# igashov/DiffLinker

Measured on NVIDIA H100. Metric: molecules/sec (T=500 denoising), higher is better.
Workload: dtype f32

## Files before the change

difflinker_b200/csrc/kernels_node_tc.cuh:

```cuda
#pragma once
#include "kernels_tc.cuh"

namespace dl {
namespace tcn {

using namespace dl::tc;

constexpr int TM = 128;
constexpr int X_LBO = TM * 16 + 16;
constexpr int X_BYTES = KC * X_LBO;
constexpr int HALF_BYTES = 8 * W_LBO;
constexpr int STAGE_BYTES = 2 * HALF_BYTES;
constexpr int BLOCK_BYTES = 2 * W_BYTES;
constexpr int N_RING = 2;
constexpr int N_OFF_WS = 4 * X_BYTES;
constexpr int N_OFF_MISC = N_OFF_WS + N_RING * STAGE_BYTES;
constexpr int N_OFF_BAR = N_OFF_MISC + 128 * 4 + 64;
constexpr int N_SMEM_BYTES = N_OFF_BAR + 64 + 1024;
static_assert(N_SMEM_BYTES <= 232448, "k_node_tc shared memory");
constexpr int NW = 8;
constexpr int W_NLOADER = NW;
constexpr int NODE_TC_THREADS = 32 * (NW + 1);

struct NodeTcArgs {
  float* h;
  const float* agg;
  const float* nm;
  const __half* w3;
  const __half* w4;
  const float *b3, *b4;
  float w3_descale, w4_descale;
  int tile_nodes;
  int proj_only;
  int n_proj;
  const __half* pw[2];
  const float* pb1[2];
  float p_descale[2];
  float* AB[2];
  float* ABmax[2];
};

__device__ __forceinline__ float pow2_scale_for(float bound) {
  float sc = 1.0f;
  if (!(bound <= F16_TARGET)) {
    const int ex = ((__float_as_int(bound) >> 23) & 0xff) - 127;
    sc = __int_as_float(max(127 + 13 - ex, 1) << 23);
  }
  return sc;
}

__device__ __forceinline__ void workers_sync() { asm volatile("bar.sync 1, %0;" ::"n"(32 * NW) : "memory"); }

__device__ __forceinline__ void store_elem(uint8_t* xhi, uint8_t* xlo, int c, int n, float v) {
  const __half hi = __float2half_rn(v);
  const __half lo = __float2half_rn(v - __half2float(hi));
  const int off = (c >> 3) * X_LBO + n * 16 + (c & 7) * 2;
  *reinterpret_cast<__half*>(xhi + off) = hi;
  *reinterpret_cast<__half*>(xlo + off) = lo;
}

__global__ void __launch_bounds__(NODE_TC_THREADS, 1) k_node_tc(int n_total, NodeTcArgs a) {
  extern __shared__ uint8_t smem_raw[];
  uint8_t* sm = smem_raw + ((1024u - (smem_u32(smem_raw) & 1023u)) & 1023u);
  const uint32_t sbase = smem_u32(sm);
  const int tid = threadIdx.x, warp = tid >> 5, lane = tid & 31;
  const int tile = a.tile_nodes > 0 ? a.tile_nodes : TM;
  const int g0 = blockIdx.x * tile;
  const int n_live = min(tile, n_total - g0);

  const uint32_t bar_full = sbase + N_OFF_BAR, bar_empty = bar_full + 8 * N_RING;
  uint8_t* xa_hi = sm; uint8_t* xa_lo = xa_hi + X_BYTES;
  uint8_t* xb_hi = sm + 2 * X_BYTES; uint8_t* xb_lo = xb_hi + X_BYTES;
  float* nms = reinterpret_cast<float*>(sm + N_OFF_MISC);
  int* tilemax = reinterpret_cast<int*>(sm + N_OFF_MISC + 512);

  if (tid == 0) {
    for (int i = 0; i < N_RING; ++i) { mbar_init(bar_full + 8 * i, 1); mbar_init(bar_empty + 8 * i, NW); }
    fence_barrier_init();
  }
  if (tid < 16) tilemax[tid] = 0;
  __syncthreads();

  const int blk0 = a.proj_only ? 3 : 0;
  const int n_blocks = 3 + 2 * a.n_proj - blk0;
  const int n_half = 2 * n_blocks;

  if (warp == W_NLOADER) {
    if (lane == 0) {
      for (int i = 0; i < n_half; ++i) {
        const int s = i % N_RING, blk = (i >> 1) + blk0, hf = i & 1;
        if (i >= N_RING) mbar_wait(bar_empty + 8 * s, ((i - N_RING) / N_RING) & 1);
        const __half* base = blk < 2 ? a.w3 + (size_t)blk * (BLOCK_BYTES / 2)
                             : blk == 2 ? a.w4
                                        : a.pw[(blk - 3) >> 1] + (size_t)((blk - 3) & 1) * (BLOCK_BYTES / 2);
        const uint8_t* src = reinterpret_cast<const uint8_t*>(base);
        const uint32_t dst = sbase + N_OFF_WS + s * STAGE_BYTES;
        mbar_expect_tx(bar_full + 8 * s, STAGE_BYTES);
        bulk_g2s(dst, src + hf * HALF_BYTES, HALF_BYTES, bar_full + 8 * s);
        bulk_g2s(dst + HALF_BYTES, src + W_BYTES + hf * HALF_BYTES, HALF_BYTES, bar_full + 8 * s);
      }
    }
    return;
  }

  chain_wait();
  if (tid == 0) chain_release();
  if (tid < TM) nms[tid] = tid < n_live ? a.nm[g0 + tid] : 0.f;

  const int g = warp >> 2, q = lane & 3;
  const int c0 = 64 * g + 16 * (warp & 3) + (lane >> 2);
  int tm_calls = 0;
  auto tile_max = [&](float mx) -> float {
#pragma unroll
    for (int o = 16; o > 0; o >>= 1) mx = fmaxf(mx, __shfl_xor_sync(0xffffffffu, mx, o));
    int* slot = tilemax + (tm_calls++ & 15);
    if (lane == 0) atomicMax(slot, __float_as_int(mx));
    workers_sync();
    return __int_as_float(*slot);
  };
  auto operand_ready = [&]() {
    fence_proxy_async();
    workers_sync();
  };
  int hb = 0;
  float d[64];
#pragma unroll
  for (int i = 0; i < 64; ++i) d[i] = 0.f;
  auto gemm = [&](const uint8_t* xop, int n_blk_half, bool accumulate) {
    for (int k = 0; k < n_blk_half; ++k, ++hb) {
      const int s = hb % N_RING, hf = hb & 1;
      mbar_wait(bar_full + 8 * s, (hb / N_RING) & 1);
      const uint32_t xh = smem_u32(xop) + (8 * hf) * X_LBO, xl = xh + X_BYTES;
      const uint32_t wh = sbase + N_OFF_WS + s * STAGE_BYTES + g * 1024, wl = wh + HALF_BYTES;
      gemm_3xf16(d, wh, wl, W_LBO, xh, xl, X_LBO, 2 * X_LBO, 4, accumulate || k > 0);
      __syncwarp();
      if (lane == 0) mbar_arrive(bar_empty + 8 * s);
    }
  };

  auto load_rows = [&](float scale) -> float {
    float mx = 0.f;
#pragma unroll 1
    for (int rb = warp; rb < TM; rb += 4 * NW) {
      float4 hv[4], av[4];
#pragma unroll
      for (int j = 0; j < 4; ++j) {
        const int r = rb + NW * j;
        hv[j] = make_float4(0, 0, 0, 0); av[j] = hv[j];
        if (r < n_live) {
          hv[j] = *reinterpret_cast<const float4*>(a.h + (size_t)(g0 + r) * H + lane * 4);
          if (!a.proj_only) av[j] = __ldg(reinterpret_cast<const float4*>(a.agg + (size_t)(g0 + r) * H + lane * 4));
        }
      }
#pragma unroll
      for (int j = 0; j < 4; ++j) {
        const int r = rb + NW * j;
        mx = fmaxf(mx, fmaxf(fmaxf(fabsf(hv[j].x), fabsf(hv[j].y)), fmaxf(fabsf(hv[j].z), fabsf(hv[j].w))));
        mx = fmaxf(mx, fmaxf(fmaxf(fabsf(av[j].x), fabsf(av[j].y)), fmaxf(fabsf(av[j].z), fabsf(av[j].w))));
        const int off = (lane >> 1) * X_LBO + r * 16 + (lane & 1) * 8;
        uint2 hi, lo;
        split2(hv[j].x * scale, hv[j].y * scale, hi.x, lo.x); split2(hv[j].z * scale, hv[j].w * scale, hi.y, lo.y);
        *reinterpret_cast<uint2*>(xa_hi + off) = hi; *reinterpret_cast<uint2*>(xa_lo + off) = lo;
        split2(av[j].x * scale, av[j].y * scale, hi.x, lo.x); split2(av[j].z * scale, av[j].w * scale, hi.y, lo.y);
        *reinterpret_cast<uint2*>(xb_hi + off) = hi; *reinterpret_cast<uint2*>(xb_lo + off) = lo;
      }
    }
    return mx;
  };

  float s1 = 1.f, s2 = 1.f, s3 = 1.f;
#pragma unroll 1
  for (int pass = 0; pass < 2; ++pass) {
    const float mx = load_rows(s1);
    if (pass == 1) break;
    s1 = pow2_scale_for(tile_max(mx));
    if (s1 == 1.0f) break;
  }
  operand_ready();

  if (a.proj_only) {
    s3 = s1;
  } else {
    gemm(xa_hi, 2, false);
    gemm(xb_hi, 2, true);
    workers_sync();
    const float2 bias3 = make_float2(__ldg(a.b3 + c0), __ldg(a.b3 + c0 + 8));
    const float ds1 = a.w3_descale / s1;
#pragma unroll 1
    for (int pass = 0; pass < 2; ++pass) {
      float mx = 0.f;
#pragma unroll
      for (int j = 0; j < 16; ++j)
#pragma unroll
        for (int u = 0; u < 4; ++u) {
          const float v = fmaf(d[4 * j + u], ds1, (u & 2) ? bias3.y : bias3.x);
          mx = fmaxf(mx, fabsf(v));
          store_elem(xb_hi, xb_lo, c0 + (u & 2) * 4, 8 * j + 2 * q + (u & 1), silu_f(v) * s2);
        }
      if (pass == 1) break;
      s2 = pow2_scale_for(tile_max(mx));
      if (s2 == 1.0f) break;
    }
    operand_ready();
    gemm(xb_hi, 2, false);
    const float2 bias4 = make_float2(__ldg(a.b4 + c0), __ldg(a.b4 + c0 + 8));
    const float ds2 = a.w4_descale / s2;
    float mx = 0.f;
#pragma unroll
    for (int j = 0; j < 16; ++j)
#pragma unroll
      for (int u = 0; u < 4; ++u) {
        const int n = 8 * j + 2 * q + (u & 1), c = c0 + (u & 2) * 4;
        float* hp = a.h + (size_t)(g0 + n) * H + c;
        const float hv = n < n_live ? *hp : 0.f;
        const float o = (hv + fmaf(d[4 * j + u], ds2, (u & 2) ? bias4.y : bias4.x)) * nms[n];
        if (n < n_live) *hp = o;
        mx = fmaxf(mx, fabsf(o));
        d[4 * j + u] = o;
        store_elem(xa_hi, xa_lo, c, n, o);
      }
    s3 = pow2_scale_for(tile_max(mx));
    if (s3 != 1.0f) {
#pragma unroll
      for (int j = 0; j < 16; ++j)
#pragma unroll
        for (int u = 0; u < 4; ++u) store_elem(xa_hi, xa_lo, c0 + (u & 2) * 4, 8 * j + 2 * q + (u & 1), d[4 * j + u] * s3);
    }
    operand_ready();
  }

  for (int p = 0; p < a.n_proj; ++p) {
#pragma unroll 1
    for (int pt = 0; pt < 2; ++pt) {
      gemm(xa_hi, 2, false);
      const float2 bias = pt == 0 ? make_float2(__ldg(a.pb1[p] + c0), __ldg(a.pb1[p] + c0 + 8)) : make_float2(0.f, 0.f);
      float* ab = a.AB[p] + (size_t)g0 * 2 * H + pt * H;
      const float ds = a.p_descale[p] / s3;
      float mx = 0.f;
#pragma unroll
      for (int j = 0; j < 16; ++j)
#pragma unroll
        for (int u = 0; u < 4; ++u) {
          const int n = 8 * j + 2 * q + (u & 1);
          const float o = fmaf(d[4 * j + u], ds, (u & 2) ? bias.y : bias.x);
          if (n < n_live) { ab[(size_t)n * 2 * H + c0 + (u & 2) * 4] = o; mx = fmaxf(mx, fabsf(o)); }
        }
      const float tmx = tile_max(mx);
      if (tid < n_live) a.ABmax[p][(size_t)(g0 + tid) * 2 + pt] = tmx;
    }
  }
}

inline size_t pack_blocks(const std::vector<float>& W, int in_stride, int nblk, std::vector<__half>& blob,
                          float* descale) {
  while (blob.size() % 64) blob.push_back(__float2half(0.f));
  const size_t off = blob.size();
  const size_t per = 2 * (size_t)KC * H * 8;
  blob.resize(off + nblk * per);
  float mx = 0.f;
  for (int c = 0; c < H; ++c)
    for (int k = 0; k < nblk * H; ++k) mx = std::max(mx, std::fabs(W[(size_t)c * in_stride + k]));
  int ex = 0;
  if (mx > 0.f && std::isfinite(mx)) { std::frexp(mx, &ex); ex -= 1; }
  const int sh = std::min(std::max(13 - ex, -40), 40);
  const float scale = std::ldexp(1.0f, sh);
  *descale = std::ldexp(1.0f, -sh);
  for (int b = 0; b < nblk; ++b)
    for (int kc = 0; kc < KC; ++kc)
      for (int c = 0; c < H; ++c)
        for (int u = 0; u < 8; ++u) {
          const float v = W[(size_t)c * in_stride + b * H + kc * 8 + u] * scale;
          const __half hi = __float2half_rn(v);
          const __half lo = __float2half_rn(v - __half2float(hi));
          blob[off + b * per + ((size_t)kc * H + c) * 8 + u] = hi;
          blob[off + b * per + (size_t)KC * H * 8 + ((size_t)kc * H + c) * 8 + u] = lo;
        }
  return off;
}

inline int pick_tile_nodes(int n, int num_sms) {
  const int per = (n + num_sms - 1) / std::max(num_sms, 1);
  return std::min(TM, std::max(8, (per + 7) & ~7));
}

inline dl_status configure_node() {
  if (cudaFuncSetAttribute(k_node_tc, cudaFuncAttributeMaxDynamicSharedMemorySize, N_SMEM_BYTES) != cudaSuccess) return DL_ERR_CUDA;
  return DL_OK;
}

inline void launch_node(int n, const NodeTcArgs& ta, cudaStream_t st) {
  const int grid = (n + ta.tile_nodes - 1) / ta.tile_nodes;
  launch_chain(k_node_tc, dim3(grid), dim3(NODE_TC_THREADS), N_SMEM_BYTES, st, n, ta);
}

}
}
```

difflinker_b200/csrc/kernels_tc.cuh:

```cuda
#pragma once
#include <cuda_fp16.h>

#include <cmath>
#include <cstdio>
#include <type_traits>
#include <vector>

#include "../../include/difflinker_b200.h"
#include "kernels_simt.cuh"

namespace dl {
namespace tc {

constexpr bool AVAILABLE = true;
constexpr int TN = 128;
constexpr int MAXR = 32;
constexpr int KC = 16;
constexpr int W_LBO = H * 16;
constexpr int B_LBO = TN * 16 + 16;
constexpr int SBO = 128;
constexpr int W_BYTES = KC * W_LBO;
constexpr int B_BYTES = KC * B_LBO;
constexpr float F16_TARGET = 16384.0f;

constexpr int N_STAGE = 2;
constexpr int N_ACC = 4;

constexpr int W_EPI = 0;
constexpr int N_EPI_WARPS = 8;
constexpr int W_LOAD = 8;
constexpr int W_TBL = 9;
constexpr int N_TBL_WARPS = 3;
constexpr int W_PROD = 12;
constexpr int N_PROD_WARPS = 8;
constexpr int EDGE_TC_THREADS = 32 * (W_PROD + N_PROD_WARPS);
constexpr int REGS_EPI = 112, REGS_CTRL = 64;
constexpr int BAR_TURN0 = 3, BAR_TURN1 = 4;

constexpr int OFF_WHI = 0;
constexpr int OFF_WLO = OFF_WHI + W_BYTES;
constexpr int OFF_ST = OFF_WLO + W_BYTES;
constexpr int STAGE_BYTES = 2 * B_BYTES;
constexpr int OFF_TBL = OFF_ST + N_STAGE * STAGE_BYTES;
constexpr int TBL_HDR = 0;
constexpr int TBL_ROWOFF = 64;
constexpr int TBL_COLOFF = TBL_ROWOFF + TN * 4;
constexpr int TBL_D = TBL_COLOFF + TN * 4;
constexpr int TBL_D0 = TBL_D + TN * 4;
constexpr int TBL_SC = TBL_D0 + TN * 4;
constexpr int TBL_EM = TBL_SC + TN * 4;
constexpr int TBL_CD = TBL_EM + TN * 8;
constexpr int TBL_ROWNODE = TBL_CD + TN * 12;
constexpr int TBL_ROWSTART = TBL_ROWNODE + MAXR * 4;
constexpr int TBL_BYTES = TBL_ROWSTART + (MAXR + 4) * 4;
constexpr int OFF_B2W5 = OFF_TBL + N_ACC * TBL_BYTES;
constexpr int OFF_TX = OFF_B2W5 + H * 8;
constexpr int OFF_BAR = OFF_TX + TN * 12;
constexpr int BAR_W = 0, BAR_FULL = 8, BAR_EMPTY = BAR_FULL + 8 * N_STAGE, BAR_TBL = BAR_EMPTY + 8 * N_STAGE,
              BAR_TEMPTY = BAR_TBL + 8 * N_ACC, BAR_END = BAR_TEMPTY + 8 * N_ACC;
constexpr int SMEM_BYTES = OFF_BAR + BAR_END + 1024;
static_assert(SMEM_BYTES <= 232448, "k_edge_tc exceeds the 227 KB of shared memory a CTA can opt into");
static_assert(TBL_BYTES % 16 == 0, "table slots must keep 16-byte alignment");

__device__ __forceinline__ uint32_t smem_u32(const void* p) { return (uint32_t)__cvta_generic_to_shared(p); }

__device__ __forceinline__ void mbar_init(uint32_t bar, uint32_t count) {
  asm volatile("mbarrier.init.shared::cta.b64 [%0], %1;" ::"r"(bar), "r"(count));
}
__device__ __forceinline__ void mbar_expect_tx(uint32_t bar, uint32_t bytes) {
  asm volatile("mbarrier.arrive.expect_tx.shared::cta.b64 _, [%0], %1;" ::"r"(bar), "r"(bytes) : "memory");
}
__device__ __constant__ int c_wait_mode = 1;
constexpr uint32_t WAIT_HINT_NS = 20000;
__device__ __forceinline__ void mbar_wait(uint32_t bar, uint32_t parity) {
  uint32_t done = 0;
  const int mode = c_wait_mode;
  if (mode == 1) {
    for (uint32_t spin = 0; spin < (1u << 20); ++spin) {
      asm volatile(
          "{\n\t.reg .pred p;\n\t"
          "mbarrier.try_wait.parity.shared::cta.b64 p, [%1], %2, %3;\n\t"
          "selp.u32 %0, 1, 0, p;\n\t}"
          : "=r"(done)
          : "r"(bar), "r"(parity), "r"(WAIT_HINT_NS)
          : "memory");
      if (done) return;
    }
    __trap();
  }
  for (uint32_t spin = 0; spin < (1u << 28); ++spin) {
    asm volatile(
        "{\n\t.reg .pred p;\n\t"
        "mbarrier.try_wait.parity.shared::cta.b64 p, [%1], %2;\n\t"
        "selp.u32 %0, 1, 0, p;\n\t}"
        : "=r"(done)
        : "r"(bar), "r"(parity)
        : "memory");
    if (done) return;
    if (mode == 2) __nanosleep(32);
  }
  __trap();
}
__device__ __forceinline__ void mbar_arrive(uint32_t bar) {
  asm volatile("mbarrier.arrive.shared::cta.b64 _, [%0];" ::"r"(bar) : "memory");
}
__device__ __forceinline__ void named_sync(int id, int nthreads) {
  asm volatile("bar.sync %0, %1;" ::"r"(id), "r"(nthreads) : "memory");
}
__device__ __forceinline__ void named_arrive(int id, int nthreads) {
  asm volatile("bar.arrive %0, %1;" ::"r"(id), "r"(nthreads) : "memory");
}
__device__ __forceinline__ void mbar_wait_relaxed(uint32_t bar, uint32_t parity) {
  uint32_t done = 0;
  for (uint32_t spin = 0; spin < (1u << 24); ++spin) {
    asm volatile(
        "{\n\t.reg .pred p;\n\t"
        "mbarrier.try_wait.parity.shared::cta.b64 p, [%1], %2;\n\t"
        "selp.u32 %0, 1, 0, p;\n\t}"
        : "=r"(done)
        : "r"(bar), "r"(parity)
        : "memory");
    if (done) return;
    __nanosleep(64);
  }
  __trap();
}
__device__ __forceinline__ void fence_barrier_init() { asm volatile("fence.mbarrier_init.release.cluster;" ::: "memory"); }
__device__ __forceinline__ void fence_proxy_async() { asm volatile("fence.proxy.async.shared::cta;" ::: "memory"); }

__device__ __forceinline__ void bulk_g2s(uint32_t dst, const void* src, uint32_t bytes, uint32_t bar) {
  asm volatile("cp.async.bulk.shared::cluster.global.mbarrier::complete_tx::bytes [%0], [%1], %2, [%3];" ::"r"(dst),
               "l"(src), "r"(bytes), "r"(bar)
               : "memory");
}

__device__ __forceinline__ uint64_t wg_desc(uint32_t saddr, uint32_t lbo, uint32_t sbo) {
  return (uint64_t)((saddr & 0x3FFFFu) >> 4) | ((uint64_t)(lbo >> 4) << 16) | ((uint64_t)(sbo >> 4) << 32);
}
__device__ __forceinline__ void wg_fence() { asm volatile("wgmma.fence.sync.aligned;" ::: "memory"); }
__device__ __forceinline__ void wg_commit() { asm volatile("wgmma.commit_group.sync.aligned;" ::: "memory"); }
__device__ __forceinline__ void wg_wait_all() { asm volatile("wgmma.wait_group.sync.aligned 0;" ::: "memory"); }
__device__ __forceinline__ void fence_acc(float (&d)[64]) {
#pragma unroll
  for (int i = 0; i < 64; ++i) asm volatile("" : "+f"(d[i])::"memory");
}
template <int TRANS_B>
__device__ __forceinline__ void wgmma_m64n128k16(float (&d)[64], uint64_t adesc, uint64_t bdesc, uint32_t accumulate) {
  asm volatile(
      "{\n\t.reg .pred p;\n\t"
      "setp.ne.b32 p, %66, 0;\n\t"
      "wgmma.mma_async.sync.aligned.m64n128k16.f32.f16.f16 "
      "{%0, %1, %2, %3, %4, %5, %6, %7, %8, %9, %10, %11, %12, %13, %14, %15, %16, %17, %18, %19, %20, %21, %22, %23, %24, %25, %26, %27, %28, %29, %30, %31, %32, %33, %34, %35, %36, %37, %38, %39, %40, %41, %42, %43, %44, %45, %46, %47, %48, %49, %50, %51, %52, %53, %54, %55, %56, %57, %58, %59, %60, %61, %62, %63}, %64, %65, p, 1, 1, 0, %67;\n\t}"
      : "+f"(d[0]), "+f"(d[1]), "+f"(d[2]), "+f"(d[3]), "+f"(d[4]), "+f"(d[5]), "+f"(d[6]), "+f"(d[7]), "+f"(d[8]), "+f"(d[9]), "+f"(d[10]), "+f"(d[11]), "+f"(d[12]), "+f"(d[13]), "+f"(d[14]), "+f"(d[15]), "+f"(d[16]), "+f"(d[17]), "+f"(d[18]), "+f"(d[19]), "+f"(d[20]), "+f"(d[21]), "+f"(d[22]), "+f"(d[23]), "+f"(d[24]), "+f"(d[25]), "+f"(d[26]), "+f"(d[27]), "+f"(d[28]), "+f"(d[29]), "+f"(d[30]), "+f"(d[31]), "+f"(d[32]), "+f"(d[33]), "+f"(d[34]), "+f"(d[35]), "+f"(d[36]), "+f"(d[37]), "+f"(d[38]), "+f"(d[39]), "+f"(d[40]), "+f"(d[41]), "+f"(d[42]), "+f"(d[43]), "+f"(d[44]), "+f"(d[45]), "+f"(d[46]), "+f"(d[47]), "+f"(d[48]), "+f"(d[49]), "+f"(d[50]), "+f"(d[51]), "+f"(d[52]), "+f"(d[53]), "+f"(d[54]), "+f"(d[55]), "+f"(d[56]), "+f"(d[57]), "+f"(d[58]), "+f"(d[59]), "+f"(d[60]), "+f"(d[61]), "+f"(d[62]), "+f"(d[63])
      : "l"(adesc), "l"(bdesc), "r"(accumulate), "n"(TRANS_B));
}
template <int TRANS_B = 0>
__device__ __forceinline__ void mma_3xf16(float (&d)[64], uint32_t a_hi, uint32_t a_lo, uint32_t a_lbo, uint32_t b_hi,
                                          uint32_t b_lo, uint32_t b_lbo, uint32_t b_ks_stride, int nks, bool accumulate) {
#pragma unroll
  for (int ks = 0; ks < nks; ++ks) {
    const uint64_t ah = wg_desc(a_hi + ks * 2 * a_lbo, a_lbo, SBO), al = wg_desc(a_lo + ks * 2 * a_lbo, a_lbo, SBO);
    const uint64_t bh = wg_desc(b_hi + ks * b_ks_stride, b_lbo, SBO), bl = wg_desc(b_lo + ks * b_ks_stride, b_lbo, SBO);
    wgmma_m64n128k16<TRANS_B>(d, al, bh, (accumulate || ks > 0) ? 1u : 0u);
    wgmma_m64n128k16<TRANS_B>(d, ah, bl, 1u);
    wgmma_m64n128k16<TRANS_B>(d, ah, bh, 1u);
  }
}
template <int TRANS_B = 0>
__device__ __forceinline__ void gemm_3xf16(float (&d)[64], uint32_t a_hi, uint32_t a_lo, uint32_t a_lbo, uint32_t b_hi,
                                           uint32_t b_lo, uint32_t b_lbo, uint32_t b_ks_stride, int nks, bool accumulate) {
  fence_acc(d);
  wg_fence();
  mma_3xf16<TRANS_B>(d, a_hi, a_lo, a_lbo, b_hi, b_lo, b_lbo, b_ks_stride, nks, accumulate);
  wg_commit();
  wg_wait_all();
  fence_acc(d);
}

__device__ __forceinline__ void split2v(float2 v, uint32_t& hi, uint32_t& lo) {
  __half2 h = __float22half2_rn(v);
  float2 back = __half22float2(h);
  __half2 l = __float22half2_rn(fadd2(v, make_float2(-back.x, -back.y)));
  hi = *reinterpret_cast<uint32_t*>(&h);
  lo = *reinterpret_cast<uint32_t*>(&l);
}
__device__ __forceinline__ void split2(float a, float b, uint32_t& hi, uint32_t& lo) {
  __half2 h = __floats2half2_rn(a, b);
  float2 back = __half22float2(h);
  __half2 l = __floats2half2_rn(a - back.x, b - back.y);
  hi = *reinterpret_cast<uint32_t*>(&h);
  lo = *reinterpret_cast<uint32_t*>(&l);
}
__device__ __forceinline__ int gcl_row_of_edge(int e) { return 8 * ((e & 31) >> 1) + 2 * (e >> 5) + (e & 1); }
struct Tile {
  int b, nc, slot0, nrt, c0, ncc;
  bool first_chunk, last_chunk;
  const int* rows;
  int Et;
  int start;
  int node;
};

template <bool COORD>
struct TileIter {
  const int4* list;
  const int* rowlist;
  int N, wi_end, wi, rt, c0, cache_base, lane;
  int4 cache;
  __device__ TileIter(const Plan& p, int N_) : N(N_), rt(0), c0(0), cache_base(-(1 << 30)), lane(threadIdx.x & 31) {
    list = COORD ? p.xitems : p.items;
    rowlist = COORD ? p.xrowidx : p.rowidx;
    const int total = COORD ? *p.n_xitems : *p.n_items;
    const int per = total / (int)gridDim.x, extra = total % (int)gridDim.x, c = (int)blockIdx.x;
    wi = c * per + min(c, extra);
    wi_end = wi + per + (c < extra ? 1 : 0);
    cache = make_int4(0, 0, 0, 0);
  }
  __device__ bool next(Tile& t) {
    while (wi < wi_end) {
      if (wi - cache_base >= 32) {
        cache_base = wi;
        cache = list[min(wi + lane, wi_end - 1)];
      }
      const int src = wi - cache_base;
      const int b = __shfl_sync(0xffffffffu, cache.x, src), r_begin = __shfl_sync(0xffffffffu, cache.y, src);
      const int r_count = __shfl_sync(0xffffffffu, cache.z, src), nc = __shfl_sync(0xffffffffu, cache.w, src);
      int per = nc >= TN ? 1 : TN / max(nc, 1);
      if (per > MAXR) per = MAXR;
      if (rt >= r_count || nc <= 0) { wi += 1; rt = 0; c0 = 0; continue; }
      t.b = b; t.nc = nc; t.slot0 = r_begin + rt; t.nrt = min(per, r_count - rt);
      t.c0 = c0; t.ncc = min(TN, nc - c0);
      t.first_chunk = c0 == 0; t.last_chunk = c0 + TN >= nc;
      t.rows = rowlist + (size_t)b * N;
      c0 += TN;
      if (c0 >= nc) { c0 = 0; rt += per; }
      return true;
    }
    return false;
  }
};

struct RecIter {
  const int* recs;
  int n, k, G, lane, cur, nxt, chunk;
  __device__ RecIter(const int* recs_, const int* n_recs) : recs(recs_), lane(threadIdx.x & 31), cur(0), chunk(0) {
    n = *n_recs; G = (int)gridDim.x; k = (int)blockIdx.x;
    nxt = k < n ? recs[(size_t)k * CUT_REC + lane] : 0;
  }
  __device__ bool next(Tile& t) {
    if (chunk == 0) {
      if (k >= n) return false;
      cur = nxt;
      const int kn = k + G;
      nxt = kn < n ? recs[(size_t)kn * CUT_REC + lane] : 0;
    }
    const int w1 = __shfl_sync(0xffffffffu, cur, 1), v2 = __shfl_sync(0xffffffffu, cur, 2);
    const int info = __shfl_sync(0xffffffffu, cur, (4 + lane) & 31);
    t.b = __shfl_sync(0xffffffffu, cur, 0);
    t.nc = 0; t.slot0 = 0; t.rows = nullptr;
    if (((w1 >> 8) & 1) == 0) {
      t.nrt = w1 & 0xff; t.Et = v2; t.ncc = v2; t.c0 = 0; t.first_chunk = true; t.last_chunk = true;
      t.node = info & 0xffff; t.start = info >> 16;
      k += G;
    } else {
      const int deg = v2, c0 = chunk * TN;
      t.nrt = 1; t.Et = min(TN, deg - c0); t.ncc = t.Et; t.c0 = c0;
      t.first_chunk = chunk == 0; t.last_chunk = c0 + TN >= deg;
      t.node = __shfl_sync(0xffffffffu, cur, 4) & 0xffff;
      t.start = lane == 0 ? 0 : t.Et;
      ++chunk;
      if (t.last_chunk) { chunk = 0; k += G; }
    }
    return true;
  }
};

template <bool COORD, bool SPARSE>
__device__ __forceinline__ typename std::conditional<SPARSE, RecIter, TileIter<COORD>>::type make_iter(const EdgeArgs& a, int N) {
  if constexpr (SPARSE) return RecIter(a.recs, a.n_recs);
  else return TileIter<COORD>(a.plan, N);
}

template <bool COORD, bool SPARSE = false, int OPT = 0>
__global__ void __launch_bounds__(EDGE_TC_THREADS, 1) k_edge_tc(Geom gm, EdgeArgs a, const __half* __restrict__ w2tc) {
  constexpr bool MEAN = (OPT & OPT_MEAN) != 0, TANH = (OPT & OPT_TANH) != 0, EMB = (OPT & OPT_SIN) != 0;
  static_assert(COORD || !TANH, "tanh only bounds the coordinate update");
  extern __shared__ uint8_t smem_raw[];
  uint8_t* sm = smem_raw + ((1024u - (smem_u32(smem_raw) & 1023u)) & 1023u);
  const uint32_t sbase = smem_u32(sm);
  const int tid = threadIdx.x, lane = tid & 31, warp = tid >> 5;
  const int N = gm.N;

  const uint32_t bars = sbase + OFF_BAR;
  float2* b2w5 = reinterpret_cast<float2*>(sm + OFF_B2W5);

  if (tid == 0) {
    mbar_init(bars + BAR_W, 1);
    for (int i = 0; i < N_STAGE; ++i) { mbar_init(bars + BAR_FULL + 8 * i, N_PROD_WARPS); mbar_init(bars + BAR_EMPTY + 8 * i, N_EPI_WARPS); }
    for (int i = 0; i < N_ACC; ++i) {
      mbar_init(bars + BAR_TBL + 8 * i, 1);
      mbar_init(bars + BAR_TEMPTY + 8 * i, N_EPI_WARPS);
    }
    fence_barrier_init();
  }
  if (tid < H) b2w5[tid] = make_float2(a.b2[tid], COORD ? a.w5[tid] : 0.f);
  __syncthreads();

  if (warp >= W_LOAD && warp < W_PROD) {
    asm volatile("setmaxnreg.dec.sync.aligned.u32 %0;" ::"n"(REGS_CTRL));
  if (warp >= W_TBL && warp < W_TBL + N_TBL_WARPS) {
    const int tw = warp - W_TBL;
    typename std::conditional<SPARSE, RecIter, TileIter<COORD>>::type iter = make_iter<COORD, SPARSE>(a, N);
    Tile cur;
    for (int t = 0;; ++t) {
      const int acc = t & (N_ACC - 1);
      const bool more = iter.next(cur);
      if (t % N_TBL_WARPS != tw) { if (!more) break; continue; }
      if (t >= N_ACC) mbar_wait_relaxed(bars + BAR_TEMPTY + 8 * acc, ((t - N_ACC) / N_ACC) & 1);
      uint8_t* tb = sm + OFF_TBL + acc * TBL_BYTES;
      int* hdr = reinterpret_cast<int*>(tb + TBL_HDR);
      if (more) {
        const int Et = SPARSE ? cur.Et : cur.nrt * cur.ncc;
        const size_t gb = (size_t)cur.b * N;
        int heavy_deg = 0;
        if constexpr (MEAN && SPARSE) {
          const int w1 = __shfl_sync(0xffffffffu, iter.cur, 1), v2 = __shfl_sync(0xffffffffu, iter.cur, 2);
          heavy_deg = ((w1 >> 8) & 1) ? v2 : 0;
        }
        if (lane == 0) {
          hdr[0] = Et; hdr[1] = cur.nrt; hdr[2] = cur.ncc;
          hdr[3] = (cur.first_chunk ? 1 : 0) | (cur.last_chunk ? 2 : 0);
          hdr[4] = cur.b;
          if (MEAN && SPARSE) hdr[6] = heavy_deg;
        }
        if (SPARSE) {
          if (lane < cur.nrt) {
            reinterpret_cast<int*>(tb + TBL_ROWNODE)[lane] = cur.node;
            reinterpret_cast<int*>(tb + TBL_ROWSTART)[lane] = cur.start;
          }
          if (lane == 0) reinterpret_cast<int*>(tb + TBL_ROWSTART)[cur.nrt] = Et;
        } else {
          if (lane < cur.nrt) {
            reinterpret_cast<int*>(tb + TBL_ROWNODE)[lane] = cur.rows[cur.slot0 + lane];
            reinterpret_cast<int*>(tb + TBL_ROWSTART)[lane] = lane * cur.ncc;
          }
          if (lane == 0) reinterpret_cast<int*>(tb + TBL_ROWSTART)[cur.nrt] = Et;
        }
        bool any_rescale = false;
#pragma unroll
        for (int e = lane; e < TN; e += 32) {
          const int ev = min(e, Et - 1);
          int i, j;
          float ew_list = 1.f;
          if (SPARSE) {
            int rr = 0;
            for (int r = 1; r < cur.nrt; ++r) rr += ev >= __shfl_sync(0xffffffffu, cur.start, r) ? 1 : 0;
            i = __shfl_sync(0xffffffffu, cur.node, rr);
            const int first_col = __shfl_sync(0xffffffffu, cur.start, rr);
            const int raw = a.nbr[(gb + i) * N + cur.c0 + (ev - first_col)];
            j = raw & 0x7fffffff;
            ew_list = raw < 0 ? 0.f : 1.f;
          } else {
            const int rr = ev / cur.ncc, jj = ev - rr * cur.ncc;
            i = cur.rows[cur.slot0 + rr];
            j = a.plan.colidx[gb + cur.c0 + jj];
          }
          const float4 xi = a.x4[gb + i], xj = a.x4[gb + j], yi = a.x04[gb + i], yj = a.x04[gb + j];
          const float dx = xi.x - xj.x, dy = xi.y - xj.y, dz = xi.z - xj.z;
          const float ex = yi.x - yj.x, ey = yi.y - yj.y, ez = yi.z - yj.z;
          float d, d0;
          if constexpr (EMB) {
            d = radial_rn(dx, dy, dz); d0 = radial_rn(ex, ey, ez);
          } else {
            d = dx * dx + dy * dy + dz * dz;
            d0 = ex * ex + ey * ey + ez * ez;
          }
          int ci = 0, cj = 0;
          if (!SPARSE && gm.graph_type != 0) { ci = a.cls[gb + i]; cj = a.cls[gb + j]; }
          reinterpret_cast<int*>(tb + TBL_ROWOFF)[e] = (int)((gb + i) * 2 * H);
          reinterpret_cast<int*>(tb + TBL_COLOFF)[e] = (int)((gb + j) * 2 * H + H);
          reinterpret_cast<float*>(tb + TBL_D)[e] = d;
          reinterpret_cast<float*>(tb + TBL_D0)[e] = d0;
          const float bound = EMB ? a.ABmax[(gb + i) * 2] + a.ABmax[(gb + j) * 2 + 1] + a.wdmax
                                  : a.ABmax[(gb + i) * 2] + a.ABmax[(gb + j) * 2 + 1] + d * a.wdmax + d0 * a.w0max;
          float sc = 1.0f;
          if (!(bound <= F16_TARGET)) {
            const int ex2 = ((__float_as_int(bound) >> 23) & 0xff) - 127;
            sc = __int_as_float(max(127 + 13 - ex2, 1) << 23);
          }
          reinterpret_cast<float*>(tb + TBL_SC)[e] = sc;
          any_rescale |= (sc != 1.0f);
          const float ew = SPARSE ? ew_list
                                  : edge_weight(gm.graph_type, a.edge_mask ? a.edge_mask + gb * N : nullptr, N, i, j, ci, cj, d0);
          reinterpret_cast<float2*>(tb + TBL_EM)[e] =
              COORD ? make_float2(ew, a.w2_descale / sc)
                    : make_float2(ew * -0.6931471805599453f, (a.w2_descale / sc) * -1.4426950408889634f);
          if (COORD) {
            const float inv = 1.0f / (sqrtf(d + 1e-8f) + gm.norm_constant);
            float* cds = reinterpret_cast<float*>(tb + TBL_CD);
            cds[e * 3 + 0] = dx * inv; cds[e * 3 + 1] = dy * inv; cds[e * 3 + 2] = dz * inv;
          }
        }
        any_rescale = __any_sync(0xffffffffu, any_rescale);
        if (lane == 0) hdr[5] = any_rescale ? 1 : 0;
      } else if (lane == 0) {
        hdr[0] = 0;
      }
      __syncwarp();
      if (lane == 0) mbar_arrive(bars + BAR_TBL + 8 * acc);
      if (!more) break;
    }
  } else if (warp == W_LOAD) {
    if (lane == 0) {
      mbar_expect_tx(bars + BAR_W, 2 * W_BYTES);
      bulk_g2s(sbase + OFF_WHI, w2tc, 2 * W_BYTES, bars + BAR_W);
    }
  }
  } else if (warp >= W_PROD) {
    const int pw = warp - W_PROD;
    const int kc = lane & 15, esub = lane >> 4;
    float2 wdr[4], w0r[4];
#pragma unroll
    for (int q = 0; q < 4; ++q) {
      wdr[q] = make_float2(__ldg(a.wd + kc * 8 + 2 * q), __ldg(a.wd + kc * 8 + 2 * q + 1));
      w0r[q] = make_float2(__ldg(a.w0 + kc * 8 + 2 * q), __ldg(a.w0 + kc * 8 + 2 * q + 1));
    }
    for (int t = 0;; ++t) {
      const int acc = t & (N_ACC - 1), s = t & (N_STAGE - 1);
      mbar_wait(bars + BAR_TBL + 8 * acc, (t / N_ACC) & 1);
      const uint8_t* tb = sm + OFF_TBL + acc * TBL_BYTES;
      const int Et = reinterpret_cast<const int*>(tb + TBL_HDR)[0];
      if (t >= N_STAGE) mbar_wait(bars + BAR_EMPTY + 8 * s, ((t - N_STAGE) / N_STAGE) & 1);
      if (Et > 0) {
        const int* rowoff = reinterpret_cast<const int*>(tb + TBL_ROWOFF);
        const int* coloff = reinterpret_cast<const int*>(tb + TBL_COLOFF);
        const float* dv = reinterpret_cast<const float*>(tb + TBL_D);
        const float* d0v = reinterpret_cast<const float*>(tb + TBL_D0);
        const float* scv = reinterpret_cast<const float*>(tb + TBL_SC);
        uint8_t* bhi = sm + OFF_ST + s * STAGE_BYTES + kc * B_LBO;
        uint8_t* blo = bhi + B_BYTES;
        const bool rescale = reinterpret_cast<const int*>(tb + TBL_HDR)[5] != 0;
        constexpr int ITEMS = TN / (2 * N_PROD_WARPS);
        float4 pa0, pa1, pb[2][2];
        const int e_base = ITEMS * (2 * pw + esub);
        int ro_cur = rowoff[e_base];
        {
          const float* ap = a.AB + ro_cur + kc * 8;
          pa0 = __ldg(reinterpret_cast<const float4*>(ap)); pa1 = __ldg(reinterpret_cast<const float4*>(ap + 4));
        }
#pragma unroll
        for (int pf = 0; pf < 2; ++pf) {
          const float* bp = a.AB + coloff[e_base + pf] + kc * 8;
          pb[pf][0] = __ldg(reinterpret_cast<const float4*>(bp)); pb[pf][1] = __ldg(reinterpret_cast<const float4*>(bp + 4));
        }
#pragma unroll
        for (int it = 0; it < ITEMS; ++it) {
          const int e = e_base + it;
          const int slot = it & 1;
          const float4 b0 = pb[slot][0], b1 = pb[slot][1];
          if (it + 2 < ITEMS) {
            const float* bp = a.AB + coloff[e + 2] + kc * 8;
            pb[slot][0] = __ldg(reinterpret_cast<const float4*>(bp)); pb[slot][1] = __ldg(reinterpret_cast<const float4*>(bp + 4));
          }
          const int ro = rowoff[e];
          if (ro != ro_cur) {
            ro_cur = ro;
            const float* ap = a.AB + ro + kc * 8;
            pa0 = __ldg(reinterpret_cast<const float4*>(ap)); pa1 = __ldg(reinterpret_cast<const float4*>(ap + 4));
          }
          const float4 a0 = pa0, a1 = pa1;
          float2 pre_emb[4];
          if constexpr (EMB) {
// ... 405 lines not shown
```

Baseline: 188.7.

## Template node tensor-core kernel on tile width to use narrower wgmma shapes

The node MLP kernel is now templated on the node-tile width NT, rounded up to a multiple of 16. Each instantiation uses a matching wgmma m64nNk16 shape, accumulator size, shared-memory layout and loop trip count. When tiles are smaller than 128 nodes this avoids tensor-core work and epilogue processing on padded columns, and it shrinks shared memory. In exchange there are eight kernel instantiations selected by recursive template dispatch, and the tile-max code now folds the bias into the scale bound for partial tiles.

```diff
diff --git a/difflinker_b200/csrc/kernels_node_tc.cuh b/difflinker_b200/csrc/kernels_node_tc.cuh
--- a/difflinker_b200/csrc/kernels_node_tc.cuh
+++ b/difflinker_b200/csrc/kernels_node_tc.cuh
@@ -7,20 +7,27 @@
 using namespace dl::tc;
 
 constexpr int TM = 128;
-constexpr int X_LBO = TM * 16 + 16;
-constexpr int X_BYTES = KC * X_LBO;
 constexpr int HALF_BYTES = 8 * W_LBO;
 constexpr int STAGE_BYTES = 2 * HALF_BYTES;
 constexpr int BLOCK_BYTES = 2 * W_BYTES;
 constexpr int N_RING = 2;
-constexpr int N_OFF_WS = 4 * X_BYTES;
-constexpr int N_OFF_MISC = N_OFF_WS + N_RING * STAGE_BYTES;
-constexpr int N_OFF_BAR = N_OFF_MISC + 128 * 4 + 64;
-constexpr int N_SMEM_BYTES = N_OFF_BAR + 64 + 1024;
-static_assert(N_SMEM_BYTES <= 232448, "k_node_tc shared memory");
 constexpr int NW = 8;
 constexpr int W_NLOADER = NW;
 constexpr int NODE_TC_THREADS = 32 * (NW + 1);
+
+template <int NT>
+struct NodeLayout {
+  static constexpr int X_LBO = NT * 16 + 16;
+  static constexpr int X_BYTES = KC * X_LBO;
+  static constexpr int OFF_WS = 4 * X_BYTES;
+  static constexpr int OFF_MISC = OFF_WS + N_RING * STAGE_BYTES;
+  static constexpr int OFF_BAR = OFF_MISC + TM * 4 + 64;
+  static constexpr int SMEM_BYTES = OFF_BAR + 64 + 1024;
+  static_assert(NT % 16 == 0 && NT >= 16 && NT <= TM, "k_node_tc widths are multiples of 16 up to 128");
+  static_assert(SMEM_BYTES <= 232448, "k_node_tc shared memory");
+};
+
+inline int node_width(int tile) { return (tile + 15) & ~15; }
 
 struct NodeTcArgs {
   float* h;
@@ -51,28 +58,32 @@
 
 __device__ __forceinline__ void workers_sync() { asm volatile("bar.sync 1, %0;" ::"n"(32 * NW) : "memory"); }
 
+template <int LBO>
 __device__ __forceinline__ void store_elem(uint8_t* xhi, uint8_t* xlo, int c, int n, float v) {
   const __half hi = __float2half_rn(v);
   const __half lo = __float2half_rn(v - __half2float(hi));
-  const int off = (c >> 3) * X_LBO + n * 16 + (c & 7) * 2;
+  const int off = (c >> 3) * LBO + n * 16 + (c & 7) * 2;
   *reinterpret_cast<__half*>(xhi + off) = hi;
   *reinterpret_cast<__half*>(xlo + off) = lo;
 }
 
+template <int NT>
 __global__ void __launch_bounds__(NODE_TC_THREADS, 1) k_node_tc(int n_total, NodeTcArgs a) {
+  using Ly = NodeLayout<NT>;
+  constexpr int X_LBO = Ly::X_LBO, X_BYTES = Ly::X_BYTES, NJ = NT / 8;
   extern __shared__ uint8_t smem_raw[];
   uint8_t* sm = smem_raw + ((1024u - (smem_u32(smem_raw) & 1023u)) & 1023u);
   const uint32_t sbase = smem_u32(sm);
   const int tid = threadIdx.x, warp = tid >> 5, lane = tid & 31;
-  const int tile = a.tile_nodes > 0 ? a.tile_nodes : TM;
+  const int tile = a.tile_nodes;
   const int g0 = blockIdx.x * tile;
   const int n_live = min(tile, n_total - g0);
 
-  const uint32_t bar_full = sbase + N_OFF_BAR, bar_empty = bar_full + 8 * N_RING;
+  const uint32_t bar_full = sbase + Ly::OFF_BAR, bar_empty = bar_full + 8 * N_RING;
   uint8_t* xa_hi = sm; uint8_t* xa_lo = xa_hi + X_BYTES;
   uint8_t* xb_hi = sm + 2 * X_BYTES; uint8_t* xb_lo = xb_hi + X_BYTES;
-  float* nms = reinterpret_cast<float*>(sm + N_OFF_MISC);
-  int* tilemax = reinterpret_cast<int*>(sm + N_OFF_MISC + 512);
+  float* nms = reinterpret_cast<float*>(sm + Ly::OFF_MISC);
+  int* tilemax = reinterpret_cast<int*>(sm + Ly::OFF_MISC + TM * 4);
 
   if (tid == 0) {
     for (int i = 0; i < N_RING; ++i) { mbar_init(bar_full + 8 * i, 1); mbar_init(bar_empty + 8 * i, NW); }
@@ -92,9 +103,9 @@
         if (i >= N_RING) mbar_wait(bar_empty + 8 * s, ((i - N_RING) / N_RING) & 1);
         const __half* base = blk < 2 ? a.w3 + (size_t)blk * (BLOCK_BYTES / 2)
                              : blk == 2 ? a.w4
-                                        : a.pw[(blk - 3) >> 1] + (size_t)((blk - 3) & 1) * (BLOCK_BYTES / 2);
+                                        : ((blk - 3) >> 1 ? a.pw[1] : a.pw[0]) + (size_t)((blk - 3) & 1) * (BLOCK_BYTES / 2);
         const uint8_t* src = reinterpret_cast<const uint8_t*>(base);
-        const uint32_t dst = sbase + N_OFF_WS + s * STAGE_BYTES;
+        const uint32_t dst = sbase + Ly::OFF_WS + s * STAGE_BYTES;
         mbar_expect_tx(bar_full + 8 * s, STAGE_BYTES);
         bulk_g2s(dst, src + hf * HALF_BYTES, HALF_BYTES, bar_full + 8 * s);
         bulk_g2s(dst + HALF_BYTES, src + W_BYTES + hf * HALF_BYTES, HALF_BYTES, bar_full + 8 * s);
@@ -123,15 +134,15 @@
     workers_sync();
   };
   int hb = 0;
-  float d[64];
-#pragma unroll
-  for (int i = 0; i < 64; ++i) d[i] = 0.f;
+  float d[NT / 2];
+#pragma unroll
+  for (int i = 0; i < NT / 2; ++i) d[i] = 0.f;
   auto gemm = [&](const uint8_t* xop, int n_blk_half, bool accumulate) {
     for (int k = 0; k < n_blk_half; ++k, ++hb) {
       const int s = hb % N_RING, hf = hb & 1;
       mbar_wait(bar_full + 8 * s, (hb / N_RING) & 1);
       const uint32_t xh = smem_u32(xop) + (8 * hf) * X_LBO, xl = xh + X_BYTES;
-      const uint32_t wh = sbase + N_OFF_WS + s * STAGE_BYTES + g * 1024, wl = wh + HALF_BYTES;
+      const uint32_t wh = sbase + Ly::OFF_WS + s * STAGE_BYTES + g * 1024, wl = wh + HALF_BYTES;
       gemm_3xf16(d, wh, wl, W_LBO, xh, xl, X_LBO, 2 * X_LBO, 4, accumulate || k > 0);
       __syncwarp();
       if (lane == 0) mbar_arrive(bar_empty + 8 * s);
@@ -141,7 +152,7 @@
   auto load_rows = [&](float scale) -> float {
     float mx = 0.f;
 #pragma unroll 1
-    for (int rb = warp; rb < TM; rb += 4 * NW) {
+    for (int rb = warp; rb < NT; rb += 4 * NW) {
       float4 hv[4], av[4];
 #pragma unroll
       for (int j = 0; j < 4; ++j) {
@@ -155,6 +166,7 @@
 #pragma unroll
       for (int j = 0; j < 4; ++j) {
         const int r = rb + NW * j;
+        if (NT % (4 * NW) != 0 && r >= NT) break;
         mx = fmaxf(mx, fmaxf(fmaxf(fabsf(hv[j].x), fabsf(hv[j].y)), fmaxf(fabsf(hv[j].z), fabsf(hv[j].w))));
         mx = fmaxf(mx, fmaxf(fmaxf(fabsf(av[j].x), fabsf(av[j].y)), fmaxf(fabsf(av[j].z), fabsf(av[j].w))));
         const int off = (lane >> 1) * X_LBO + r * 16 + (lane & 1) * 8;
@@ -186,16 +198,17 @@
     workers_sync();
     const float2 bias3 = make_float2(__ldg(a.b3 + c0), __ldg(a.b3 + c0 + 8));
     const float ds1 = a.w3_descale / s1;
+    const float bias_mx = n_live < TM ? fmaxf(fabsf(bias3.x), fabsf(bias3.y)) : 0.f;
 #pragma unroll 1
     for (int pass = 0; pass < 2; ++pass) {
-      float mx = 0.f;
-#pragma unroll
-      for (int j = 0; j < 16; ++j)
+      float mx = bias_mx;
+#pragma unroll
+      for (int j = 0; j < NJ; ++j)
 #pragma unroll
         for (int u = 0; u < 4; ++u) {
           const float v = fmaf(d[4 * j + u], ds1, (u & 2) ? bias3.y : bias3.x);
           mx = fmaxf(mx, fabsf(v));
-          store_elem(xb_hi, xb_lo, c0 + (u & 2) * 4, 8 * j + 2 * q + (u & 1), silu_f(v) * s2);
+          store_elem<X_LBO>(xb_hi, xb_lo, c0 + (u & 2) * 4, 8 * j + 2 * q + (u & 1), silu_f(v) * s2);
         }
       if (pass == 1) break;
       s2 = pow2_scale_for(tile_max(mx));
@@ -207,7 +220,7 @@
     const float ds2 = a.w4_descale / s2;
     float mx = 0.f;
 #pragma unroll
-    for (int j = 0; j < 16; ++j)
+    for (int j = 0; j < NJ; ++j)
 #pragma unroll
       for (int u = 0; u < 4; ++u) {
         const int n = 8 * j + 2 * q + (u & 1), c = c0 + (u & 2) * 4;
@@ -217,19 +230,22 @@
         if (n < n_live) *hp = o;
         mx = fmaxf(mx, fabsf(o));
         d[4 * j + u] = o;
-        store_elem(xa_hi, xa_lo, c, n, o);
+        store_elem<X_LBO>(xa_hi, xa_lo, c, n, o);
       }
     s3 = pow2_scale_for(tile_max(mx));
     if (s3 != 1.0f) {
 #pragma unroll
-      for (int j = 0; j < 16; ++j)
-#pragma unroll
-        for (int u = 0; u < 4; ++u) store_elem(xa_hi, xa_lo, c0 + (u & 2) * 4, 8 * j + 2 * q + (u & 1), d[4 * j + u] * s3);
+      for (int j = 0; j < NJ; ++j)
+#pragma unroll
+        for (int u = 0; u < 4; ++u)
+          store_elem<X_LBO>(xa_hi, xa_lo, c0 + (u & 2) * 4, 8 * j + 2 * q + (u & 1), d[4 * j + u] * s3);
     }
     operand_ready();
   }
 
-  for (int p = 0; p < a.n_proj; ++p) {
+#pragma unroll
+  for (int p = 0; p < 2; ++p) {
+    if (p == 1 && a.n_proj < 2) break;
 #pragma unroll 1
     for (int pt = 0; pt < 2; ++pt) {
       gemm(xa_hi, 2, false);
@@ -238,7 +254,7 @@
       const float ds = a.p_descale[p] / s3;
       float mx = 0.f;
 #pragma unroll
-      for (int j = 0; j < 16; ++j)
+      for (int j = 0; j < NJ; ++j)
 #pragma unroll
         for (int u = 0; u < 4; ++u) {
           const int n = 8 * j + 2 * q + (u & 1);
@@ -283,15 +299,22 @@
   return std::min(TM, std::max(8, (per + 7) & ~7));
 }
 
-inline dl_status configure_node() {
-  if (cudaFuncSetAttribute(k_node_tc, cudaFuncAttributeMaxDynamicSharedMemorySize, N_SMEM_BYTES) != cudaSuccess) return DL_ERR_CUDA;
-  return DL_OK;
-}
-
-inline void launch_node(int n, const NodeTcArgs& ta, cudaStream_t st) {
+template <int NT = 16>
+dl_status configure_node() {
+  if (cudaFuncSetAttribute(k_node_tc<NT>, cudaFuncAttributeMaxDynamicSharedMemorySize, NodeLayout<NT>::SMEM_BYTES) != cudaSuccess)
+    return DL_ERR_CUDA;
+  if constexpr (NT < TM) return configure_node<NT + 16>();
+  else return DL_OK;
+}
+
+template <int NT = 16>
+void launch_node(int n, const NodeTcArgs& ta, cudaStream_t st) {
+  if constexpr (NT < TM) {
+    if (node_width(ta.tile_nodes) > NT) { launch_node<NT + 16>(n, ta, st); return; }
+  }
   const int grid = (n + ta.tile_nodes - 1) / ta.tile_nodes;
-  launch_chain(k_node_tc, dim3(grid), dim3(NODE_TC_THREADS), N_SMEM_BYTES, st, n, ta);
-}
-
-}
-}
+  launch_chain(k_node_tc<NT>, dim3(grid), dim3(NODE_TC_THREADS), NodeLayout<NT>::SMEM_BYTES, st, n, ta);
+}
+
+}
+}
diff --git a/difflinker_b200/csrc/kernels_tc.cuh b/difflinker_b200/csrc/kernels_tc.cuh
--- a/difflinker_b200/csrc/kernels_tc.cuh
+++ b/difflinker_b200/csrc/kernels_tc.cuh
@@ -140,9 +140,10 @@
 __device__ __forceinline__ void wg_fence() { asm volatile("wgmma.fence.sync.aligned;" ::: "memory"); }
 __device__ __forceinline__ void wg_commit() { asm volatile("wgmma.commit_group.sync.aligned;" ::: "memory"); }
 __device__ __forceinline__ void wg_wait_all() { asm volatile("wgmma.wait_group.sync.aligned 0;" ::: "memory"); }
-__device__ __forceinline__ void fence_acc(float (&d)[64]) {
-#pragma unroll
-  for (int i = 0; i < 64; ++i) asm volatile("" : "+f"(d[i])::"memory");
+template <int NR>
+__device__ __forceinline__ void fence_acc(float (&d)[NR]) {
+#pragma unroll
+  for (int i = 0; i < NR; ++i) asm volatile("" : "+f"(d[i])::"memory");
 }
 template <int TRANS_B>
 __device__ __forceinline__ void wgmma_m64n128k16(float (&d)[64], uint64_t adesc, uint64_t bdesc, uint32_t accumulate) {
@@ -154,20 +155,72 @@
       : "+f"(d[0]), "+f"(d[1]), "+f"(d[2]), "+f"(d[3]), "+f"(d[4]), "+f"(d[5]), "+f"(d[6]), "+f"(d[7]), "+f"(d[8]), "+f"(d[9]), "+f"(d[10]), "+f"(d[11]), "+f"(d[12]), "+f"(d[13]), "+f"(d[14]), "+f"(d[15]), "+f"(d[16]), "+f"(d[17]), "+f"(d[18]), "+f"(d[19]), "+f"(d[20]), "+f"(d[21]), "+f"(d[22]), "+f"(d[23]), "+f"(d[24]), "+f"(d[25]), "+f"(d[26]), "+f"(d[27]), "+f"(d[28]), "+f"(d[29]), "+f"(d[30]), "+f"(d[31]), "+f"(d[32]), "+f"(d[33]), "+f"(d[34]), "+f"(d[35]), "+f"(d[36]), "+f"(d[37]), "+f"(d[38]), "+f"(d[39]), "+f"(d[40]), "+f"(d[41]), "+f"(d[42]), "+f"(d[43]), "+f"(d[44]), "+f"(d[45]), "+f"(d[46]), "+f"(d[47]), "+f"(d[48]), "+f"(d[49]), "+f"(d[50]), "+f"(d[51]), "+f"(d[52]), "+f"(d[53]), "+f"(d[54]), "+f"(d[55]), "+f"(d[56]), "+f"(d[57]), "+f"(d[58]), "+f"(d[59]), "+f"(d[60]), "+f"(d[61]), "+f"(d[62]), "+f"(d[63])
       : "l"(adesc), "l"(bdesc), "r"(accumulate), "n"(TRANS_B));
 }
-template <int TRANS_B = 0>
-__device__ __forceinline__ void mma_3xf16(float (&d)[64], uint32_t a_hi, uint32_t a_lo, uint32_t a_lbo, uint32_t b_hi,
+#define DL_WG_R0 "%0, %1, %2, %3, %4, %5, %6, %7"
+#define DL_WG_R1 ", %8, %9, %10, %11, %12, %13, %14, %15"
+#define DL_WG_R2 ", %16, %17, %18, %19, %20, %21, %22, %23"
+#define DL_WG_R3 ", %24, %25, %26, %27, %28, %29, %30, %31"
+#define DL_WG_R4 ", %32, %33, %34, %35, %36, %37, %38, %39"
+#define DL_WG_R5 ", %40, %41, %42, %43, %44, %45, %46, %47"
+#define DL_WG_R6 ", %48, %49, %50, %51, %52, %53, %54, %55"
+#define DL_WG_D(i) "+f"(d[i]), "+f"(d[i + 1]), "+f"(d[i + 2]), "+f"(d[i + 3]), "+f"(d[i + 4]), "+f"(d[i + 5]), "+f"(d[i + 6]), "+f"(d[i + 7])
+#define DL_WG_STR(x) #x
+#define DL_WGMMA_NARROW(N, REGS, A, B, P, T, ...)                                                                      \
+  template <int TRANS_B>                                                                                               \
+  __device__ __forceinline__ void wgmma_m64n##N##k16(float (&d)[N / 2], uint64_t adesc, uint64_t bdesc, uint32_t accumulate) { \
+    asm volatile("{\n\t.reg .pred p;\n\tsetp.ne.b32 p, %" DL_WG_STR(P) ", 0;\n\t"                                     \
+                 "wgmma.mma_async.sync.aligned.m64n" DL_WG_STR(N) "k16.f32.f16.f16 {" REGS "}, %" DL_WG_STR(A)         \
+                 ", %" DL_WG_STR(B) ", p, 1, 1, 0, %" DL_WG_STR(T) ";\n\t}"                                            \
+                 : __VA_ARGS__                                                                                         \
+                 : "l"(adesc), "l"(bdesc), "r"(accumulate), "n"(TRANS_B));                                             \
+  }
+DL_WGMMA_NARROW(16, DL_WG_R0, 8, 9, 10, 11, DL_WG_D(0))
+DL_WGMMA_NARROW(32, DL_WG_R0 DL_WG_R1, 16, 17, 18, 19, DL_WG_D(0), DL_WG_D(8))
+DL_WGMMA_NARROW(48, DL_WG_R0 DL_WG_R1 DL_WG_R2, 24, 25, 26, 27, DL_WG_D(0), DL_WG_D(8), DL_WG_D(16))
+DL_WGMMA_NARROW(64, DL_WG_R0 DL_WG_R1 DL_WG_R2 DL_WG_R3, 32, 33, 34, 35, DL_WG_D(0), DL_WG_D(8), DL_WG_D(16), DL_WG_D(24))
+DL_WGMMA_NARROW(80, DL_WG_R0 DL_WG_R1 DL_WG_R2 DL_WG_R3 DL_WG_R4, 40, 41, 42, 43, DL_WG_D(0), DL_WG_D(8), DL_WG_D(16),
+                DL_WG_D(24), DL_WG_D(32))
+DL_WGMMA_NARROW(96, DL_WG_R0 DL_WG_R1 DL_WG_R2 DL_WG_R3 DL_WG_R4 DL_WG_R5, 48, 49, 50, 51, DL_WG_D(0), DL_WG_D(8),
+                DL_WG_D(16), DL_WG_D(24), DL_WG_D(32), DL_WG_D(40))
+DL_WGMMA_NARROW(112, DL_WG_R0 DL_WG_R1 DL_WG_R2 DL_WG_R3 DL_WG_R4 DL_WG_R5 DL_WG_R6, 56, 57, 58, 59, DL_WG_D(0), DL_WG_D(8),
+                DL_WG_D(16), DL_WG_D(24), DL_WG_D(32), DL_WG_D(40), DL_WG_D(48))
+#undef DL_WGMMA_NARROW
+#undef DL_WG_STR
+#undef DL_WG_D
+#undef DL_WG_R0
+#undef DL_WG_R1
+#undef DL_WG_R2
+#undef DL_WG_R3
+#undef DL_WG_R4
+#undef DL_WG_R5
+#undef DL_WG_R6
+template <int TRANS_B, int NR>
+__device__ __forceinline__ void wgmma_k16(float (&d)[NR], uint64_t adesc, uint64_t bdesc, uint32_t accumulate) {
+  if constexpr (NR == 64) wgmma_m64n128k16<TRANS_B>(d, adesc, bdesc, accumulate);
+  else if constexpr (NR == 56) wgmma_m64n112k16<TRANS_B>(d, adesc, bdesc, accumulate);
+  else if constexpr (NR == 48) wgmma_m64n96k16<TRANS_B>(d, adesc, bdesc, accumulate);
+  else if constexpr (NR == 40) wgmma_m64n80k16<TRANS_B>(d, adesc, bdesc, accumulate);
+  else if constexpr (NR == 32) wgmma_m64n64k16<TRANS_B>(d, adesc, bdesc, accumulate);
+  else if constexpr (NR == 24) wgmma_m64n48k16<TRANS_B>(d, adesc, bdesc, accumulate);
+  else if constexpr (NR == 16) wgmma_m64n32k16<TRANS_B>(d, adesc, bdesc, accumulate);
+  else {
+    static_assert(NR == 8, "wgmma N must be a multiple of 16 up to 128");
+    wgmma_m64n16k16<TRANS_B>(d, adesc, bdesc, accumulate);
+  }
+}
+template <int TRANS_B = 0, int NR = 64>
+__device__ __forceinline__ void mma_3xf16(float (&d)[NR], uint32_t a_hi, uint32_t a_lo, uint32_t a_lbo, uint32_t b_hi,
                                           uint32_t b_lo, uint32_t b_lbo, uint32_t b_ks_stride, int nks, bool accumulate) {
 #pragma unroll
   for (int ks = 0; ks < nks; ++ks) {
     const uint64_t ah = wg_desc(a_hi + ks * 2 * a_lbo, a_lbo, SBO), al = wg_desc(a_lo + ks * 2 * a_lbo, a_lbo, SBO);
     const uint64_t bh = wg_desc(b_hi + ks * b_ks_stride, b_lbo, SBO), bl = wg_desc(b_lo + ks * b_ks_stride, b_lbo, SBO);
-    wgmma_m64n128k16<TRANS_B>(d, al, bh, (accumulate || ks > 0) ? 1u : 0u);
-    wgmma_m64n128k16<TRANS_B>(d, ah, bl, 1u);
-    wgmma_m64n128k16<TRANS_B>(d, ah, bh, 1u);
-  }
-}
-template <int TRANS_B = 0>
-__device__ __forceinline__ void gemm_3xf16(float (&d)[64], uint32_t a_hi, uint32_t a_lo, uint32_t a_lbo, uint32_t b_hi,
+    wgmma_k16<TRANS_B>(d, al, bh, (accumulate || ks > 0) ? 1u : 0u);
+    wgmma_k16<TRANS_B>(d, ah, bl, 1u);
+    wgmma_k16<TRANS_B>(d, ah, bh, 1u);
+  }
+}
+template <int TRANS_B = 0, int NR = 64>
+__device__ __forceinline__ void gemm_3xf16(float (&d)[NR], uint32_t a_hi, uint32_t a_lo, uint32_t a_lbo, uint32_t b_hi,
                                            uint32_t b_lo, uint32_t b_lbo, uint32_t b_ks_stride, int nks, bool accumulate) {
   fence_acc(d);
   wg_fence();
```

Result: faster. 193.5, median of 6 (+2.5%).
